# netease-youdao/EmotiVoice

Measured on AMD Instinct MI355X. Metric: mel_frames_per_sec, higher is better.
Workload: dtype f16+mxfp4 (fp32-class activations travelling as plane sets; per product one fp16 MFMA on the hi parts + two block-scaled MFMAs for the cross terms: fp4 x fp4 in every generator stage, the decoder's conv-FFN and QKV / output projections, fp4 weights x E5M2 activations in the fused 32-channel k = 3 pa

## Files before the change

emotivoice_amd/csrc/ev_gemm.hip:

```cpp
#include <hip/hip_fp16.h>
#include <stdlib.h>

#include "ev_kernels.h"
#include "ev_mxq.h"

#pragma clang fp contract(off)

namespace ev {

typedef _Float16 half8 __attribute__((ext_vector_type(8)));
typedef float f32x4 __attribute__((ext_vector_type(4)));
typedef float f32x2 __attribute__((ext_vector_type(2)));
typedef _Float16 half2v __attribute__((ext_vector_type(2)));

static constexpr int MAX_SPAN = 64;

__device__ __forceinline__ float max_raw(float a, float b) {
    float r;
    asm("v_max_f32 %0, %1, %2" : "=v"(r) : "v"(a), "v"(b));
    return r;
}
__device__ __forceinline__ float min_raw(float a, float b) {
    float r;
    asm("v_min_f32 %0, %1, %2" : "=v"(r) : "v"(a), "v"(b));
// ... 1933 lines not shown
                else asm volatile("" :: "v"(o.x), "v"(o.y), "v"(o.z), "v"(o.w));
            }
        }
        vmask = vmask_next;
        EV_PAIR_SYNC()
        cur ^= 1;
    }
#undef EV_PAIR_GLOAD
#undef EV_PAIR_SSTORE
#undef EV_PAIR_ROW
#undef EV_PAIR_VROW
#undef EV_PAIR_VLOAD
#undef EV_PAIR_VMASK
}

static size_t pair_lds_bytes(int k, bool twob = false) {
    if (twob) return 2 * (size_t)k * 32 * 64 + 2 * 320 * 64 + 272 * 64;
    return 2 * (size_t)k * 32 * 64 + 2 * 384 * 64 + 272 * 64 + 8 * 32 * (32 * 4 + 16);
}
static constexpr size_t PAIR64_LDS_BYTES = 2 * 2 * (size_t)(3 * 64 * 64) + 2 * 2 * (size_t)(272 * 64) + 2 * (size_t)(272 * 64);

static int g_n_cu[64];
static bool g_dev_ready[64];
static int current_device() { int d = 0; (void)hipGetDevice(&d); return (d >= 0 && d < 64) ? d : 0; }

static int device_cus() {
    const int d = current_device();
    if (!g_dev_ready[d]) (void)init_device_kernels(d);
    return g_n_cu[d] > 0 ? g_n_cu[d] : 256;
}

void launch_resblock_pair_c32(const ResPairParams& p, hipStream_t s) {
    const int n_cu = device_cus();
    const int h2 = (p.k - 1) / 2, bmo = 256 - 2 * h2;
    const int ntiles = (p.M + bmo - 1) / bmo;
    const int grid = ntiles < n_cu ? ntiles : n_cu;
    static const char* one_env = tuning_env("EV_PAIR_1B");
    const bool twob = p.k <= 3 && !(one_env && one_env[0] == '1') && !(p.epi.reserved0 & 4) && ntiles >= 4 * n_cu;
    const size_t lds = pair_lds_bytes(p.k, twob);
    const int grid2 = ntiles < 2 * n_cu ? ntiles : 2 * n_cu;
#define EV_PAIR_LAUNCH(KK, TB, G)                                                                                          \
        if (p.epi.add16_a) hipLaunchKernelGGL((resblock_pair_c32_kernel<KK, 2, TB>), dim3(G), dim3(512), lds, s, p);  \
        else if (p.epi.acc32) hipLaunchKernelGGL((resblock_pair_c32_kernel<KK, 1, TB>), dim3(G), dim3(512), lds, s, p); \
        else hipLaunchKernelGGL((resblock_pair_c32_kernel<KK, 0, TB>), dim3(G), dim3(512), lds, s, p);
    switch (p.k) {
        case 3: if (twob) { EV_PAIR_LAUNCH(3, true, grid2) } else { EV_PAIR_LAUNCH(3, false, grid) } break;
        case 7: EV_PAIR_LAUNCH(7, false, grid) break;
        case 11: EV_PAIR_LAUNCH(11, false, grid) break;
        default: break;
    }
#undef EV_PAIR_LAUNCH
}

template <int K, int ACCMODE>
__global__ __launch_bounds__(512, 1) void resblock_pair_c64_kernel(const ResPairParams p) {
    constexpr int C = 64, H2 = (K - 1) / 2, BMO = 256 - 2 * H2;
    constexpr int XROWS = 272, PLANE = XROWS * 64, XBYTES = 2 * PLANE;
    constexpr int WPL = K * C * 64, WBYTES = 2 * WPL;
    constexpr int EPITCH = C * 4 + 16, EBYTES = 16 * EPITCH;
    constexpr int XCH = (XROWS * 8 + 511) / 512;
    static_assert(8 * EBYTES <= XBYTES && 256 + 2 * 5 * H2 + 2 * H2 <= XROWS && XCH == 5, "LDS aliasing / slab geometry");
    extern __shared__ __attribute__((aligned(16))) char smem[];
    char* W1s = smem;
    char* W2s = smem + WBYTES;
    char* Xa = smem + 2 * WBYTES;
    char* Xt = Xa + 2 * XBYTES;
    const int tid = threadIdx.x, lane = tid & 63, wave = tid >> 6;
    const int fr = lane & 15, fq = lane >> 4;
    const int h1 = H2 * p.dil;
    const int x_pitch = p.ldx * 2;
    const char* xg = reinterpret_cast<const char*>(p.x);
    const int ntiles = (p.M + BMO - 1) / BMO;
    const ConvGemmParams& e = p.epi;
    const int gmin = p.gmax ? p.gmin : 0, gmax = p.gmax ? p.gmax : p.M;

    for (int c = tid; c < K * C * 8; c += 512) {
        const int row = c >> 3, q = c & 7, tap = row >> 6, co = row & 63, plane = q >> 2, part = q & 3;
        const long off = ((long)(co * K + tap) * C) * 2 + q * 16;
        *reinterpret_cast<uint4*>(W1s + plane * WPL + swz(row, part)) = *reinterpret_cast<const uint4*>(reinterpret_cast<const char*>(p.w1) + off);
        *reinterpret_cast<uint4*>(W2s + plane * WPL + swz(row, part)) = *reinterpret_cast<const uint4*>(reinterpret_cast<const char*>(p.w2) + off);
    }
    f32x2 b1v[4][2];
#pragma unroll
    for (int a = 0; a < 4; ++a)
#pragma unroll
        for (int q = 0; q < 2; ++q) b1v[a][q] = f32x2{p.b1[a * 16 + 4 * fq + 2 * q], p.b1[a * 16 + 4 * fq + 2 * q + 1]};
    const int er = lane >> 3, eg = lane & 7, eco = eg * 8;
    const unsigned frbit = 1u << fr, erbit = 1u << er;
    f32x2 b2v[4];
#pragma unroll
    for (int q = 0; q < 4; ++q) b2v[q] = e.bias ? f32x2{e.bias[eco + 2 * q], e.bias[eco + 2 * q + 1]} : f32x2{0.f, 0.f};
    const f32x2 out_scale2 = f32x2{e.out_scale, e.out_scale};
    const bool has_post = e.post_lrelu != 0;
    const f32x2 post_slope2 = f32x2{e.post_slope, e.post_slope};
    const f32x2 slope01 = f32x2{0.1f, 0.1f};
    __half* const o16 = reinterpret_cast<__half*>(e.out16);
    float* const o32a = e.out32_before_post ? e.out32 : nullptr;
    float* const o32b = e.out32_before_post ? nullptr : e.out32;
    char* const trash = g_store_trash + lane * 64;

    const uint8_t* vptr = e.row_valid ? e.row_valid : g_row_always_valid;
    const int vshift = e.row_valid ? e.valid_shift : 31;
#define EV_P64_VROW(TILE) ((TILE) * BMO - H2 + wave * 32 + lane)
#define EV_P64_VLOAD(TILE, DST) { const int g_ = EV_P64_VROW(TILE); DST = vptr[min(max(g_, gmin), gmax - 1) >> vshift]; }
#define EV_P64_VMASK(TILE, SRC) __builtin_amdgcn_ballot_w64((SRC) != 0 && EV_P64_VROW(TILE) >= gmin && EV_P64_VROW(TILE) < gmax)

    uint4 xr[XCH];
    const int xrow = tid >> 3, xq = tid & 7;
    const char* const xgt = xg + xq * 16;
    const int xdst = (xq >> 2) * PLANE + swz(xrow, xq & 3);
    const bool has5 = wave < 2;
#define EV_P64_GLOAD(TILE)                                                                                 \
    {                                                                                                      \
        const int g0_ = (TILE) * BMO - H2 - h1 + xrow;                                                     \
        _Pragma("unroll") for (int i = 0; i < 4; ++i)                                                      \
            xr[i] = *reinterpret_cast<const uint4*>(xgt + (long)min(g0_ + 64 * i, gmax + 63) * x_pitch);    \
        if (has5) xr[4] = *reinterpret_cast<const uint4*>(xgt + (long)min(g0_ + 256, gmax + 63) * x_pitch); \
    }
#define EV_P64_SSTORE(BUF)                                                                                 \
    {                                                                                                      \
        _Pragma("unroll") for (int i = 0; i < 4; ++i)                                                      \
            *reinterpret_cast<uint4*>(Xa + (BUF) * XBYTES + xdst + i * 4096) = lrelu_h8(xr[i], 0.1f);      \
        if (has5) *reinterpret_cast<uint4*>(Xa + (BUF) * XBYTES + xdst + 4 * 4096) = lrelu_h8(xr[4], 0.1f); \
    }

    int tile = blockIdx.x;
    unsigned long long vmask;
    {
        uint8_t vb;
        EV_P64_GLOAD(tile)
        EV_P64_VLOAD(tile, vb)
        EV_P64_SSTORE(0)
        vmask = EV_P64_VMASK(tile, vb);
    }
    __syncthreads();
    int cur = 0;
    const int wrow0 = wave * 32 + fr;
    for (; tile < ntiles; tile += gridDim.x) {
        const int next = min(tile + (int)gridDim.x, ntiles - 1);
        const int m0 = tile * BMO;
        const int t_end = min(m0 + BMO, p.M);
        uint4 resv[2][2];
        float4 accin[2][2][2];
#pragma unroll
        for (int b = 0; b < 2; ++b)
#pragma unroll
            for (int it = 0; it < 2; ++it) {
                const int t = min(m0 + wave * 32 + b * 16 + it * 8 + er, t_end - 1);
                resv[b][it] = *reinterpret_cast<const uint4*>(xg + (long)t * x_pitch + eg * 16);
                if constexpr (ACCMODE == 1) {
                    const float* ap = e.acc32 + (long)t * e.ldacc + eco;
                    accin[b][it][0] = *reinterpret_cast<const float4*>(ap);
                    accin[b][it][1] = *reinterpret_cast<const float4*>(ap + 4);
                }
                if constexpr (ACCMODE == 2) {
                    *reinterpret_cast<uint4*>(&accin[b][it][0]) = *reinterpret_cast<const uint4*>(reinterpret_cast<const __half*>(e.add16_a) + (long)t * e.ldadd + eco);
                    *reinterpret_cast<uint4*>(&accin[b][it][1]) = *reinterpret_cast<const uint4*>(reinterpret_cast<const __half*>(e.add16_b) + (long)t * e.ldadd + eco);
                }
            }
        uint8_t vb_next;
        EV_P64_GLOAD(next)
        EV_P64_VLOAD(next, vb_next)
        __builtin_amdgcn_sched_barrier(0);
        f32x4 acc[4][2];
#pragma unroll
        for (int a = 0; a < 4; ++a)
#pragma unroll
            for (int b = 0; b < 2; ++b) acc[a][b] = f32x4{0.f, 0.f, 0.f, 0.f};
        {
            const char* Xb = Xa + cur * XBYTES;
#pragma unroll
            for (int t = 0; t < K; ++t) {
                const int r0 = wrow0 + t * p.dil;
                const int xo = r0 * 64 + ((fq ^ ((r0 >> 1) & 3)) << 4);
#pragma unroll
                for (int kc = 0; kc < 2; ++kc) {
                    uint4 xf[2], wf[4];
#pragma unroll
                    for (int b = 0; b < 2; ++b) xf[b] = *reinterpret_cast<const uint4*>(Xb + kc * PLANE + xo + b * 16 * 64);
#pragma unroll
                    for (int a = 0; a < 4; ++a) wf[a] = *reinterpret_cast<const uint4*>(W1s + kc * WPL + swz(t * 64 + a * 16 + fr, fq));
#pragma unroll
                    for (int a = 0; a < 4; ++a)
#pragma unroll
                        for (int b = 0; b < 2; ++b)
                            acc[a][b] = __builtin_amdgcn_mfma_f32_16x16x32_f16(*reinterpret_cast<half8*>(&wf[a]),
                                                                               *reinterpret_cast<half8*>(&xf[b]), acc[a][b], 0, 0, 0);
                }
            }
        }
        const unsigned xtmask = (unsigned)vmask;
#pragma unroll
        for (int b = 0; b < 2; ++b) {
            const int r1 = wrow0 + b * 16;
            const bool valid = (xtmask & (frbit << (b * 16))) != 0u;
#pragma unroll
            for (int a = 0; a < 4; ++a) {
                const f32x2 lo = lrelu2(f32x2{acc[a][b][0], acc[a][b][1]} + b1v[a][0], slope01);
                const f32x2 hi = lrelu2(f32x2{acc[a][b][2], acc[a][b][3]} + b1v[a][1], slope01);
                uint2 w;
                *reinterpret_cast<half2v*>(&w.x) = __builtin_convertvector(lo, half2v);
                *reinterpret_cast<half2v*>(&w.y) = __builtin_convertvector(hi, half2v);
                w.x = valid ? w.x : 0u; w.y = valid ? w.y : 0u;
                const int c32 = (a & 1) * 16 + 4 * fq;
                *reinterpret_cast<uint2*>(Xt + (a >> 1) * PLANE + swz(r1, c32 >> 3) + (c32 & 7) * 2) = w;
            }
        }
        __syncthreads();
#pragma unroll
        for (int a = 0; a < 4; ++a)
#pragma unroll
            for (int b = 0; b < 2; ++b) acc[a][b] = f32x4{0.f, 0.f, 0.f, 0.f};
#pragma unroll
        for (int t = 0; t < K; ++t) {
            const int r0 = wrow0 + t;
            const int xo = r0 * 64 + ((fq ^ ((r0 >> 1) & 3)) << 4);
#pragma unroll
            for (int kc = 0; kc < 2; ++kc) {
                uint4 xf[2], wf[4];
#pragma unroll
                for (int b = 0; b < 2; ++b) xf[b] = *reinterpret_cast<const uint4*>(Xt + kc * PLANE + xo + b * 16 * 64);
#pragma unroll
                for (int a = 0; a < 4; ++a) wf[a] = *reinterpret_cast<const uint4*>(W2s + kc * WPL + swz(t * 64 + a * 16 + fr, fq));
#pragma unroll
                for (int a = 0; a < 4; ++a)
#pragma unroll
                    for (int b = 0; b < 2; ++b)
                        acc[a][b] = __builtin_amdgcn_mfma_f32_16x16x32_f16(*reinterpret_cast<half8*>(&wf[a]),
                                                                           *reinterpret_cast<half8*>(&xf[b]), acc[a][b], 0, 0, 0);
            }
        }
        __builtin_amdgcn_sched_barrier(0);
        EV_P64_SSTORE(cur ^ 1)
        const unsigned long long vmask_next = EV_P64_VMASK(next, vb_next);
        char* es = Xa + cur * XBYTES + wave * EBYTES;
        const unsigned outmask = (unsigned)(vmask >> H2);
#pragma unroll
        for (int b = 0; b < 2; ++b) {
            __builtin_amdgcn_wave_barrier();
#pragma unroll
            for (int a = 0; a < 4; ++a)
                *reinterpret_cast<f32x4*>(es + fr * EPITCH + (a * 16 + 4 * fq) * 4) = acc[a][b];
            __builtin_amdgcn_wave_barrier();
#pragma unroll
            for (int it = 0; it < 2; ++it) {
                const int lr = it * 8 + er;
                const int t = m0 + wave * 32 + b * 16 + lr;
                const bool rowok = t < t_end;
                const bool valid = (outmask & (erbit << (b * 16 + it * 8))) != 0u;
                const f32x4 v0 = *reinterpret_cast<const f32x4*>(es + lr * EPITCH + eg * 32);
                const f32x4 v1 = *reinterpret_cast<const f32x4*>(es + lr * EPITCH + eg * 32 + 16);
                f32x2 v[4] = {f32x2{v0[0], v0[1]}, f32x2{v0[2], v0[3]}, f32x2{v1[0], v1[1]}, f32x2{v1[2], v1[3]}};
                const half2v* hh = reinterpret_cast<const half2v*>(&resv[b][it]);
#pragma unroll
                for (int q = 0; q < 4; ++q) v[q] = (v[q] + b2v[q] + __builtin_convertvector(hh[q], f32x2)) * out_scale2;
                if constexpr (ACCMODE == 1) {
                    v[0] += f32x2{accin[b][it][0].x, accin[b][it][0].y}; v[1] += f32x2{accin[b][it][0].z, accin[b][it][0].w};
                    v[2] += f32x2{accin[b][it][1].x, accin[b][it][1].y}; v[3] += f32x2{accin[b][it][1].z, accin[b][it][1].w};
                }
                if constexpr (ACCMODE == 2) {
                    const half2v* ha = reinterpret_cast<const half2v*>(&accin[b][it][0]);
                    const half2v* hb = reinterpret_cast<const half2v*>(&accin[b][it][1]);
#pragma unroll
                    for (int q = 0; q < 4; ++q) v[q] += __builtin_convertvector(ha[q], f32x2) + __builtin_convertvector(hb[q], f32x2);
                }
                if (o32a) {
                    float* op = rowok ? o32a + (long)t * e.ldo + eco : reinterpret_cast<float*>(trash);
                    *reinterpret_cast<float4*>(op) = valid ? make_float4(v[0][0], v[0][1], v[1][0], v[1][1]) : make_float4(0.f, 0.f, 0.f, 0.f);
                    *reinterpret_cast<float4*>(op + 4) = valid ? make_float4(v[2][0], v[2][1], v[3][0], v[3][1]) : make_float4(0.f, 0.f, 0.f, 0.f);
                }
                if (has_post) {
#pragma unroll
                    for (int q = 0; q < 4; ++q) v[q] = lrelu2(v[q], post_slope2);
                }
                if (o32b) {
                    float* op = rowok ? o32b + (long)t * e.ldo + eco : reinterpret_cast<float*>(trash);
                    *reinterpret_cast<float4*>(op) = valid ? make_float4(v[0][0], v[0][1], v[1][0], v[1][1]) : make_float4(0.f, 0.f, 0.f, 0.f);
                    *reinterpret_cast<float4*>(op + 4) = valid ? make_float4(v[2][0], v[2][1], v[3][0], v[3][1]) : make_float4(0.f, 0.f, 0.f, 0.f);
                }
                if (o16) {
                    uint4 o;
                    half2v* h = reinterpret_cast<half2v*>(&o);
#pragma unroll
                    for (int q = 0; q < 4; ++q) h[q] = __builtin_convertvector(v[q], half2v);
                    o.x = valid ? o.x : 0u; o.y = valid ? o.y : 0u; o.z = valid ? o.z : 0u; o.w = valid ? o.w : 0u;
                    *reinterpret_cast<uint4*>(rowok ? reinterpret_cast<char*>(o16 + (long)t * e.ldo + eco) : trash) = o;
                }
            }
        }
        vmask = vmask_next;
        __syncthreads();
        cur ^= 1;
    }
#undef EV_P64_GLOAD
#undef EV_P64_SSTORE
#undef EV_P64_VROW
#undef EV_P64_VLOAD
#undef EV_P64_VMASK
}

#include "ev_gemm_mx.h"
#include "ev_gemm_mx64.h"
#include "ev_pair_mx.h"
#include "ev_pair_e5.h"

#include "ev_conv64_mx.h"
#include "ev_pair64_mx.h"

int init_device_kernels(int device) {
    if (device < 0 || device >= 64) return -1;
    hipDeviceProp_t prop;
    if (hipGetDeviceProperties(&prop, device) != hipSuccess) return -1;
    g_n_cu[device] = prop.multiProcessorCount > 0 ? prop.multiProcessorCount : 256;
    hipError_t e = hipSuccess;
    auto attr = [&](const void* fn, size_t bytes) { const hipError_t r = hipFuncSetAttribute(fn, hipFuncAttributeMaxDynamicSharedMemorySize, (int)bytes); if (r != hipSuccess) e = r; };
#define EV_PAIR_ATTR(KK, TB)                                                             \
    attr((const void*)resblock_pair_c32_kernel<KK, 0, TB>, pair_lds_bytes(KK, TB));      \
    attr((const void*)resblock_pair_c32_kernel<KK, 1, TB>, pair_lds_bytes(KK, TB));      \
    attr((const void*)resblock_pair_c32_kernel<KK, 2, TB>, pair_lds_bytes(KK, TB));
    EV_PAIR_ATTR(3, false) EV_PAIR_ATTR(7, false) EV_PAIR_ATTR(11, false) EV_PAIR_ATTR(3, true)
#undef EV_PAIR_ATTR
    attr((const void*)resblock_pair_c64_kernel<3, 0>, PAIR64_LDS_BYTES);
    attr((const void*)resblock_pair_c64_kernel<3, 1>, PAIR64_LDS_BYTES);
    attr((const void*)resblock_pair_c64_kernel<3, 2>, PAIR64_LDS_BYTES);
    if (x3_set_attributes() != hipSuccess) e = hipErrorInvalidValue;
    if (phased_set_attributes() != hipSuccess) e = hipErrorInvalidValue;
    if (mx_set_attributes() != hipSuccess) e = hipErrorInvalidValue;
    if (mx64_set_attributes() != hipSuccess) e = hipErrorInvalidValue;
    if (pair_mx_set_attributes() != hipSuccess) e = hipErrorInvalidValue;
    if (pair_e5_set_attributes() != hipSuccess) e = hipErrorInvalidValue;
    if (conv64_mx_set_attributes() != hipSuccess) e = hipErrorInvalidValue;
    if (pair64_mx_set_attributes() != hipSuccess) e = hipErrorInvalidValue;
    g_dev_ready[device] = (e == hipSuccess);
    return e == hipSuccess ? 0 : -1;
}
int launch_resblock_pair_c32_mx(const ResPairParams& p, hipStream_t s) {
    const ConvGemmParams& e = p.epi;
    if (!p.w1_mx || !p.w2_mx || !e.out32 || e.out16 || e.add16_a || e.post_lrelu || e.seq_bias || e.mxo_h || !(p.k == 3 || p.k == 7 || p.k == 11) ||
        (p.k - 1) / 2 * (p.dil + 1) * 2 + 256 > 320 || p.ldx != 32) return -1;
    const int n_cu = device_cus();
    const int h2 = (p.k - 1) / 2;
    if (!(e.reserved0 & 16) && (p.k == 3 || (e.reserved0 & 32))) {
        const int bmo2 = 128 - 2 * h2, ntiles2 = (p.M + bmo2 - 1) / bmo2;
        const int grid2 = (ntiles2 + 1) / 2 < n_cu ? (ntiles2 + 1) / 2 : n_cu;
#define EV_PE5_LAUNCH(KK)                                                                                                           \
        if (e.acc32) hipLaunchKernelGGL((resblock_pair_c32_e5_kernel<KK, 1>), dim3(grid2), dim3(512), PairE5Geom<KK>::TOTAL, s, p);   \
        else hipLaunchKernelGGL((resblock_pair_c32_e5_kernel<KK, 0>), dim3(grid2), dim3(512), PairE5Geom<KK>::TOTAL, s, p);
        switch (p.k) {
            case 3: EV_PE5_LAUNCH(3) break;
            case 7: EV_PE5_LAUNCH(7) break;
            default: EV_PE5_LAUNCH(11) break;
        }
#undef EV_PE5_LAUNCH
        return 0;
    }
    {
        const int bmo2 = 128 - 2 * h2, ntiles2 = (p.M + bmo2 - 1) / bmo2;
        if (!(e.reserved0 & 4) && ntiles2 >= 2) {
            const int grid2 = (ntiles2 + 1) / 2 < n_cu ? (ntiles2 + 1) / 2 : n_cu;
#define EV_PMX2_LAUNCH(KK)                                                                                                          \
            if (e.acc32) hipLaunchKernelGGL((resblock_pair_c32_mx2_kernel<KK, 1>), dim3(grid2), dim3(512), PairMx2Geom<KK>::TOTAL, s, p);   \
            else hipLaunchKernelGGL((resblock_pair_c32_mx2_kernel<KK, 0>), dim3(grid2), dim3(512), PairMx2Geom<KK>::TOTAL, s, p);
            switch (p.k) {
                case 3: EV_PMX2_LAUNCH(3) break;
                case 7: EV_PMX2_LAUNCH(7) break;
                default: EV_PMX2_LAUNCH(11) break;
            }
#undef EV_PMX2_LAUNCH
            return 0;
        }
    }
    const int bmo = 256 - 2 * h2;
    const int ntiles = (p.M + bmo - 1) / bmo;
    const int grid = ntiles < n_cu ? ntiles : n_cu;
#define EV_PMX_LAUNCH(KK)                                                                                                         \
        if (e.acc32) hipLaunchKernelGGL((resblock_pair_c32_mx_kernel<KK, 1>), dim3(grid), dim3(512), PairMxGeom<KK>::TOTAL, s, p);   \
        else hipLaunchKernelGGL((resblock_pair_c32_mx_kernel<KK, 0>), dim3(grid), dim3(512), PairMxGeom<KK>::TOTAL, s, p);
    switch (p.k) {
        case 3: EV_PMX_LAUNCH(3) break;
        case 7: EV_PMX_LAUNCH(7) break;
        default: EV_PMX_LAUNCH(11) break;
    }
#undef EV_PMX_LAUNCH
    return 0;
}

void launch_resblock_pair_c64(const ResPairParams& p, hipStream_t s) {
    const size_t bytes = PAIR64_LDS_BYTES;
    const int n_cu = device_cus();
    const int bmo = 256 - 2;
    const int ntiles = (p.M + bmo - 1) / bmo;
    const int grid = ntiles < n_cu ? ntiles : n_cu;
    if (p.epi.add16_a) hipLaunchKernelGGL((resblock_pair_c64_kernel<3, 2>), dim3(grid), dim3(512), bytes, s, p);
    else if (p.epi.acc32) hipLaunchKernelGGL((resblock_pair_c64_kernel<3, 1>), dim3(grid), dim3(512), bytes, s, p);
    else hipLaunchKernelGGL((resblock_pair_c64_kernel<3, 0>), dim3(grid), dim3(512), bytes, s, p);
}

int mx_launch_kind(const ConvGemmParams& p) {
    if (p.dtype != DT_MX) return 0;
    return (mx64_eligible(p) || conv64_mx_eligible(p)) ? 2 : (mx_eligible(p) ? 1 : 0);
}

int splitk_check(const ConvGemmParams& p) {
    if (p.ksplit <= 1) return 0;
    if (p.dtype != DT_F32S || p.ksplit > 16 || p.N % 64 || p.K % 32 || (p.K / 32) % p.ksplit || p.M % 128 || p.add16_a || (!p.out32 && !p.out16)) return -1;
    if (!p.mx_scratch || ((uintptr_t)p.mx_scratch & 15) || p.mx_scratch_size < (size_t)p.ksplit * (size_t)p.M * (size_t)p.N * 4) return -1;
    return 0;
}

void launch_conv_gemm(const ConvGemmParams& p, hipStream_t s) {
    (void)device_cus();
    if (p.dtype == DT_F16) launch_dt<_Float16>(p, s);
    else if (p.dtype == DT_F32S) launch_split(p, s);
    else if (p.dtype == DT_MX) {
        if (mx64_eligible(p)) launch_mx64(p, s);
        else if (conv64_mx_eligible(p)) launch_conv64_mx(p, s);
        else if (mx_eligible(p)) launch_mx(p, s);
        else { ConvGemmParams q = p; q.dtype = DT_F32S; launch_split(q, s); }
    } else launch_dt<float>(p, s);
}

}
```

Measured before the change: 722,000.

## Add register-resident-weight fused resblock pair kernel for k=11 (and opt-in k=7)

Adds a new fused two-conv resblock kernel for 32-channel k=11 (and k=7 behind a flag). Each wave holds its fp16 hi-part weights in registers, and for k<=7 the fp4 cross-term weights too, instead of rereading them from LDS. The two conv stages are split across wave groups with double-buffered LDS tiles, so the second conv overlaps the first conv of the next tile. It trades higher register pressure and a fixed 256-row tile for fewer LDS weight reads, and replaces the previous mx2 path for k=11 by default.

After: 728,200, median of 6. About the same (+0.9%).

```diff
diff --git a/emotivoice_amd/csrc/ev_gemm.hip b/emotivoice_amd/csrc/ev_gemm.hip
--- a/emotivoice_amd/csrc/ev_gemm.hip
+++ b/emotivoice_amd/csrc/ev_gemm.hip
@@ -2259,6 +2259,7 @@
 #include "ev_gemm_mx.h"
 #include "ev_gemm_mx64.h"
 #include "ev_pair_mx.h"
+#include "ev_pair_regw.h"
 #include "ev_pair_e5.h"
 
 #include "ev_conv64_mx.h"
@@ -2285,6 +2286,7 @@
     if (mx_set_attributes() != hipSuccess) e = hipErrorInvalidValue;
     if (mx64_set_attributes() != hipSuccess) e = hipErrorInvalidValue;
     if (pair_mx_set_attributes() != hipSuccess) e = hipErrorInvalidValue;
+    if (pair_regw_set_attributes() != hipSuccess) e = hipErrorInvalidValue;
     if (pair_e5_set_attributes() != hipSuccess) e = hipErrorInvalidValue;
     if (conv64_mx_set_attributes() != hipSuccess) e = hipErrorInvalidValue;
     if (pair64_mx_set_attributes() != hipSuccess) e = hipErrorInvalidValue;
@@ -2311,6 +2313,16 @@
 #undef EV_PE5_LAUNCH
         return 0;
     }
+    if (!(e.reserved0 & (4 | 8 | 64)) && (p.k == 11 || (p.k == 7 && (e.reserved0 & 128)))) {
+        const int bmo = 256 - 2 * h2, ntiles = (p.M + bmo - 1) / bmo;
+        const int grid = ntiles < n_cu ? ntiles : n_cu;
+#define EV_PRW_LAUNCH(KK)                                                                                                           \
+        if (e.acc32) hipLaunchKernelGGL((resblock_pair_c32_regw_kernel<KK, 1, PairRwCfg<KK>::WQREG>), dim3(grid), dim3(512), (PairRwGeom<KK, PairRwCfg<KK>::WQREG>::TOTAL), s, p);   \
+        else hipLaunchKernelGGL((resblock_pair_c32_regw_kernel<KK, 0, PairRwCfg<KK>::WQREG>), dim3(grid), dim3(512), (PairRwGeom<KK, PairRwCfg<KK>::WQREG>::TOTAL), s, p);
+        if (p.k == 7) { EV_PRW_LAUNCH(7) } else { EV_PRW_LAUNCH(11) }
+#undef EV_PRW_LAUNCH
+        return 0;
+    }
     {
         const int bmo2 = 128 - 2 * h2, ntiles2 = (p.M + bmo2 - 1) / bmo2;
         if (!(e.reserved0 & 4) && ntiles2 >= 2) {
diff --git a/emotivoice_amd/csrc/ev_pair_regw.h b/emotivoice_amd/csrc/ev_pair_regw.h
--- /dev/null
+++ b/emotivoice_amd/csrc/ev_pair_regw.h
@@ -0,0 +1,349 @@
+#pragma once
+
+template <int K, bool WQREG>
+struct PairRwGeom {
+    static constexpr int C = 32, H2 = (K - 1) / 2, BMO = 256 - 2 * H2, KG = (K + 3) / 4, KP = KG * 4;
+    static constexpr int XR = 320, TR = 272, EPITCH = C * 4 + 16;
+    static constexpr int WQB = KP * C * 16, WSB = KP * C;
+    static constexpr int XB = XR * 64 + 2 * XR * 16 + 2 * XR;
+    static constexpr int TB = TR * 64 + 2 * TR * 16 + 2 * TR;
+    static constexpr int OFF_WQ = 0, OFF_WS = WQREG ? 0 : 4 * WQB, OFF_X = WQREG ? 0 : 4 * WQB + 4 * WSB;
+    static constexpr int OFF_T = OFF_X + 2 * XB, OFF_ES = OFF_T + 2 * TB;
+    static constexpr int TOTAL = OFF_ES + 4 * 16 * EPITCH;
+    static_assert(OFF_X % 16 == 0 && XB % 16 == 0 && TB % 16 == 0 && OFF_ES % 16 == 0 && TOTAL <= 160 * 1024 && 256 + K - 1 <= TR, "LDS plan");
+};
+
+template <int K, int ACCMODE, bool WQREG>
+__global__ __launch_bounds__(512, 1) void resblock_pair_c32_regw_kernel(const ResPairParams p) {
+    using G = PairRwGeom<K, WQREG>;
+    constexpr int C = G::C, H2 = G::H2, BMO = G::BMO, KG = G::KG, XR = G::XR, TR = G::TR, EPITCH = G::EPITCH;
+    extern __shared__ __attribute__((aligned(16))) char smem[];
+    const int tid = threadIdx.x, lane = tid & 63;
+    const int wave = __builtin_amdgcn_readfirstlane(tid >> 6);
+    const int gi = wave >> 2, lw = wave & 3, ltid = tid & 255;
+    const int fr = lane & 15, fq = lane >> 4;
+    const int dil = p.dil, h1 = H2 * dil;
+    const int x_pitch = p.ldx * 4;
+    const char* xg = reinterpret_cast<const char*>(p.x);
+    const int ntiles = (p.M + BMO - 1) / BMO;
+    const ConvGemmParams& e = p.epi;
+    const int gmin = p.gmax ? p.gmin : 0, gmax = p.gmax ? p.gmax : p.M;
+#define EV_PRW_XH(buf) (smem + G::OFF_X + (buf) * G::XB)
+#define EV_PRW_TH(buf) (smem + G::OFF_T + (buf) * G::TB)
+
+    const char* const whg = reinterpret_cast<const char*>(gi ? p.w2 : p.w1);
+    const char* const wmg = reinterpret_cast<const char*>(gi ? p.w2_mx : p.w1_mx);
+    uint4 wh[K][2];
+#pragma unroll
+    for (int t = 0; t < K; ++t)
+#pragma unroll
+        for (int a = 0; a < 2; ++a) wh[t][a] = *reinterpret_cast<const uint4*>(whg + ((long)((a * 16 + fr) * K + t) * C) * 2 + fq * 16);
+    uint4 wq[WQREG ? KG : 1][2][2];
+    int ws[WQREG ? KG : 1][2][2];
+    if constexpr (WQREG) {
+#pragma unroll
+        for (int g = 0; g < KG; ++g)
+#pragma unroll
+            for (int pl = 0; pl < 2; ++pl)
+#pragma unroll
+                for (int a = 0; a < 2; ++a) {
+                    const int wrow = (4 * g + fq) * 32 + a * 16 + fr;
+                    wq[g][pl][a] = *reinterpret_cast<const uint4*>(wmg + pl * G::WQB + wrow * 16);
+                    ws[g][pl][a] = *reinterpret_cast<const uint8_t*>(wmg + 2 * G::WQB + pl * G::WSB + wrow);
+                }
+    } else {
+        char* const Wq = smem + G::OFF_WQ;
+        char* const Wsc = smem + G::OFF_WS;
+        for (int c = tid; c < 2 * G::WQB / 16; c += 512) {
+            *reinterpret_cast<uint4*>(Wq + c * 16) = *reinterpret_cast<const uint4*>(reinterpret_cast<const char*>(p.w1_mx) + c * 16);
+            *reinterpret_cast<uint4*>(Wq + 2 * G::WQB + c * 16) = *reinterpret_cast<const uint4*>(reinterpret_cast<const char*>(p.w2_mx) + c * 16);
+        }
+        for (int c = tid; c < 2 * G::WSB / 16; c += 512) {
+            *reinterpret_cast<uint4*>(Wsc + c * 16) = *reinterpret_cast<const uint4*>(reinterpret_cast<const char*>(p.w1_mx) + 2 * G::WQB + c * 16);
+            *reinterpret_cast<uint4*>(Wsc + 2 * G::WSB + c * 16) = *reinterpret_cast<const uint4*>(reinterpret_cast<const char*>(p.w2_mx) + 2 * G::WQB + c * 16);
+        }
+    }
+    const f32x2 slope01 = f32x2{0.1f, 0.1f};
+    const uint8_t* vptr = e.row_valid ? e.row_valid : g_row_always_valid;
+    const int vshift = e.row_valid ? e.valid_shift : 31;
+#define EV_PRW_VLOAD(G0, DST) { const int g_ = (G0) + lane; DST = vptr[min(max(g_, gmin), gmax - 1) >> vshift]; }
+#define EV_PRW_VMASK(G0, SRC) __builtin_amdgcn_ballot_w64((SRC) != 0 && (G0) + lane >= gmin && (G0) + lane < gmax)
+
+#define EV_PRW_CONV(XH, NR, DIL, MID)                                                                         \
+    {                                                                                                      \
+        const int wrow0 = (int)vlane((unsigned)wrow0_inv);           \
+        const char* const xq_base_ = (XH) + (NR) * 64;                                                     \
+        const char* const xs_base_ = xq_base_ + 2 * (NR) * 16;                                             \
+        uint4 xf_[2][4];           \
+        _Pragma("unroll") for (int b = 0; b < 4; ++b)                                                      \
+            xf_[0][b] = *reinterpret_cast<const uint4*>((XH) + wrow0 * 64 + ((fq ^ ((wrow0 >> 1) & 3)) << 4) + b * 16 * 64); \
+        _Pragma("unroll") for (int t = 0; t < K; ++t) {                                                    \
+            if (t + 1 < K) {                                                                               \
+                const int r0 = wrow0 + (t + 1) * (DIL);                                                    \
+                const char* xp = (XH) + r0 * 64 + ((fq ^ ((r0 >> 1) & 3)) << 4);                           \
+                _Pragma("unroll") for (int b = 0; b < 4; ++b) xf_[(t + 1) & 1][b] = *reinterpret_cast<const uint4*>(xp + b * 16 * 64); \
+            }                                                                                              \
+            _Pragma("unroll") for (int b = 0; b < 4; ++b)                                                  \
+                _Pragma("unroll") for (int a = 0; a < 2; ++a)                                              \
+                    acc[a][b] = __builtin_amdgcn_mfma_f32_16x16x32_f16(*reinterpret_cast<half8*>(&wh[t][a]), *reinterpret_cast<half8*>(&xf_[t & 1][b]), acc[a][b], 0, 0, 0); \
+            __builtin_amdgcn_sched_barrier(0);                                                             \
+        }                                                                                                  \
+        MID                                                                                                \
+        __builtin_amdgcn_sched_barrier(0);                                                                 \
+        _Pragma("unroll") for (int g = 0; g < KG; ++g) {                                                   \
+            const int tw = 4 * g + fq;                      \
+            const int rq = wrow0 + min(tw, K - 1) * (DIL);  \
+            _Pragma("unroll") for (int pl = 0; pl < 2; ++pl) {                                             \
+                uint4 wq_[2], xq_[4];                                                                      \
+                int ws_[2], xs_[4];                                                                        \
+                _Pragma("unroll") for (int a = 0; a < 2; ++a) {                                            \
+                    if constexpr (WQREG) { wq_[a] = wq[g][pl][a]; ws_[a] = ws[g][pl][a]; }                 \
+                    else {                                                                                 \
+                        wq_[a] = *reinterpret_cast<const uint4*>(smem + G::OFF_WQ + (gi * 2 + pl) * G::WQB + (tw * 32 + a * 16 + fr) * 16); \
+                        ws_[a] = *reinterpret_cast<const uint8_t*>(smem + G::OFF_WS + (gi * 2 + pl) * G::WSB + tw * 32 + a * 16 + fr); \
+                    }                                                                                      \
+                }                                                                                          \
+                _Pragma("unroll") for (int b = 0; b < 4; ++b) {                                            \
+                    xq_[b] = *reinterpret_cast<const uint4*>(xq_base_ + pl * (NR) * 16 + (rq + b * 16) * 16); \
+                    xs_[b] = *reinterpret_cast<const uint8_t*>(xs_base_ + pl * (NR) + rq + b * 16);        \
+                }                                                                                          \
+                _Pragma("unroll") for (int b = 0; b < 4; ++b)                                              \
+                    _Pragma("unroll") for (int a = 0; a < 2; ++a)                                          \
+                        mfma_mx_inplace(acc[a][b], wq_[a], xq_[b], ws_[a], xs_[b]);                        \
+                __builtin_amdgcn_sched_barrier(0);                                                         \
+            }                                                                                              \
+        }                                                                                                  \
+        mfma_asm_fence(acc);                 \
+    }
+#define EV_PRW_BARRIER()                                         \
+    {                                                            \
+        asm volatile("s_waitcnt lgkmcnt(0)" ::: "memory");       \
+        __builtin_amdgcn_sched_barrier(0);                       \
+        __builtin_amdgcn_s_barrier();                            \
+        __builtin_amdgcn_sched_barrier(0);                       \
+    }
+
+    const int niter = (ntiles - (int)blockIdx.x + (int)gridDim.x - 1) / (int)gridDim.x;
+    const int wrow0_inv = lw * 64 + fr;
+
+    if (gi == 0) {
+        f32x2 b1v[2][2];
+#pragma unroll
+        for (int a = 0; a < 2; ++a)
+#pragma unroll
+            for (int q = 0; q < 2; ++q) b1v[a][q] = f32x2{p.b1[a * 16 + 4 * fq + 2 * q], p.b1[a * 16 + 4 * fq + 2 * q + 1]};
+        float4 xr[5][2];
+        const int xq = ltid & 3, xrow = ltid >> 2;
+        const char* const xgt = xg + xq * 32;
+        const bool need5 = lw * 16 < (K - 1) * dil;
+#define EV_PRW_ROW(G_) min((G_), gmax + 63)
+#define EV_PRW_GLOAD(TILE)                                                                                 \
+        _Pragma("unroll") for (int i = 0; i < 5; ++i) if (i < 4 || need5) {                                \
+            const char* q_ = xgt + (long)EV_PRW_ROW((TILE) * BMO - H2 - h1 + xrow + 64 * i) * x_pitch;     \
+            xr[i][0] = *reinterpret_cast<const float4*>(q_); xr[i][1] = *reinterpret_cast<const float4*>(q_ + 16); \
+        }
+#define EV_PRW_SSTORE(BUF)                                                                                 \
+        {                                                                                                  \
+            char* const Xh_ = EV_PRW_XH(BUF);                                                              \
+            char* const Xq_ = Xh_ + XR * 64;                                                               \
+            char* const Xs_ = Xq_ + 2 * XR * 16;                                                           \
+            const int xrow_ = (int)vlane((unsigned)xrow);           \
+            _Pragma("unroll") for (int i = 0; i < 5; ++i) if (i < 4 || need5) {                            \
+                const int drow_ = xrow_ + 64 * i;                                                          \
+                f32x2 a_[4] = {lrelu2(f32x2{xr[i][0].x, xr[i][0].y}, slope01), lrelu2(f32x2{xr[i][0].z, xr[i][0].w}, slope01), \
+                               lrelu2(f32x2{xr[i][1].x, xr[i][1].y}, slope01), lrelu2(f32x2{xr[i][1].z, xr[i][1].w}, slope01)}; \
+                uint4 ho_; unsigned ch_, cl_, bh_, bl_;                                                    \
+                mx_quant8(a_, ho_, ch_, cl_, bh_, bl_);                                                    \
+                *reinterpret_cast<uint4*>(Xh_ + swz(drow_, xq)) = ho_;                                     \
+                *reinterpret_cast<unsigned*>(Xq_ + drow_ * 16 + xq * 4) = ch_;                             \
+                *reinterpret_cast<unsigned*>(Xq_ + XR * 16 + drow_ * 16 + xq * 4) = cl_;                   \
+                if (xq == 0) { Xs_[drow_] = (char)bh_; Xs_[XR + drow_] = (char)bl_; }                      \
+                __builtin_amdgcn_sched_barrier(0);           \
+            }                                                                                              \
+        }
+        const unsigned long long frbit = 1ull << fr;
+        int tile = blockIdx.x;
+        unsigned long long vmask;
+        {
+            uint8_t vb;
+            EV_PRW_GLOAD(tile)
+            EV_PRW_VLOAD(tile * BMO - H2 + lw * 64, vb)
+            EV_PRW_SSTORE(0)
+            vmask = EV_PRW_VMASK(tile * BMO - H2 + lw * 64, vb);
+        }
+        EV_PRW_BARRIER()
+        for (int it_ = 0; it_ < niter; ++it_, tile += (int)gridDim.x) {
+            const int buf = it_ & 1;
+            const int next = min(tile + (int)gridDim.x, ntiles - 1);
+            uint8_t vb_next;
+#define EV_PRW_A_MID int next_ = next; asm volatile("" : "+s"(next_)); EV_PRW_GLOAD(next_) EV_PRW_VLOAD(next_ * BMO - H2 + lw * 64, vb_next)
+            f32x4 acc[2][4];
+#pragma unroll
+            for (int a = 0; a < 2; ++a)
+#pragma unroll
+                for (int b = 0; b < 4; ++b) acc[a][b] = f32x4{0.f, 0.f, 0.f, 0.f};
+            EV_PRW_CONV(EV_PRW_XH(buf), XR, dil, EV_PRW_A_MID)
+#undef EV_PRW_A_MID
+            char* const Th = EV_PRW_TH(buf);
+            char* const Tq = Th + TR * 64;
+            char* const Tsc = Tq + 2 * TR * 16;
+            const int wrow0 = (int)vlane((unsigned)wrow0_inv);
+            const bool xt_masked = vmask != ~0ull;
+#pragma unroll
+            for (int b = 0; b < 4; ++b) {
+                const int r1 = wrow0 + b * 16;
+                const bool valid = (vmask & (frbit << (b * 16))) != 0ull;
+                f32x2 v[2][2];
+                half2v hh[2][2];
+                f32x2 hf[2][2], lf[2][2];
+                float mh = 0.f, ml = 0.f;
+#pragma unroll
+                for (int a = 0; a < 2; ++a) {
+                    v[a][0] = lrelu2(f32x2{acc[a][b][0], acc[a][b][1]} + b1v[a][0], slope01);
+                    v[a][1] = lrelu2(f32x2{acc[a][b][2], acc[a][b][3]} + b1v[a][1], slope01);
+#pragma unroll
+                    for (int q = 0; q < 2; ++q) {
+                        if (xt_masked) { v[a][q][0] = valid ? v[a][q][0] : 0.f; v[a][q][1] = valid ? v[a][q][1] : 0.f; }
+                        hh[a][q] = __builtin_convertvector(v[a][q], half2v);
+                        hf[a][q] = __builtin_convertvector(hh[a][q], f32x2);
+                        lf[a][q] = v[a][q] - hf[a][q];
+                        mh = max3_abs_raw(hf[a][q][0], hf[a][q][1], mh);
+                        ml = max3_abs_raw(lf[a][q][0], lf[a][q][1], ml);
+                    }
+                }
+                mh = max_xor16_raw(max_xor32_raw(mh));
+                ml = max_xor16_raw(max_xor32_raw(ml));
+                const unsigned bh = mx_scale_byte(mh), bl = mx_scale_byte(ml);
+                const float sh = __uint_as_float(bh << 23), sl = __uint_as_float(bl << 23);
+#pragma unroll
+                for (int a = 0; a < 2; ++a) {
+                    uint2 w;
+                    w.x = *reinterpret_cast<unsigned*>(&hh[a][0]); w.y = *reinterpret_cast<unsigned*>(&hh[a][1]);
+                    const int co = a * 16 + 4 * fq;
+                    *reinterpret_cast<uint2*>(Th + swz(r1, co >> 3) + (co & 7) * 2) = w;
+                    unsigned ch = 0, cl = 0;
+                    ch = __builtin_amdgcn_cvt_scalef32_pk_fp4_f32(ch, hf[a][0][0], hf[a][0][1], sh, 0);
+                    ch = __builtin_amdgcn_cvt_scalef32_pk_fp4_f32(ch, hf[a][1][0], hf[a][1][1], sh, 1);
+                    cl = __builtin_amdgcn_cvt_scalef32_pk_fp4_f32(cl, lf[a][0][0], lf[a][0][1], sl, 0);
+                    cl = __builtin_amdgcn_cvt_scalef32_pk_fp4_f32(cl, lf[a][1][0], lf[a][1][1], sl, 1);
+                    *reinterpret_cast<unsigned short*>(Tq + r1 * 16 + (co >> 1)) = (unsigned short)ch;
+                    *reinterpret_cast<unsigned short*>(Tq + TR * 16 + r1 * 16 + (co >> 1)) = (unsigned short)cl;
+                }
+                if (fq == 0) { Tsc[r1] = (char)bh; Tsc[TR + r1] = (char)bl; }
+                __builtin_amdgcn_sched_barrier(0);
+            }
+            EV_PRW_SSTORE(buf ^ 1)
+            vmask = EV_PRW_VMASK(next * BMO - H2 + lw * 64, vb_next);
+            EV_PRW_BARRIER()
+        }
+#undef EV_PRW_SSTORE
+#undef EV_PRW_GLOAD
+#undef EV_PRW_ROW
+    } else {
+        char* const es = smem + G::OFF_ES + lw * 16 * EPITCH;
+        const int er = lane >> 2, eg = lane & 3, eco = eg * 8;
+        f32x2 b2v[4];
+#pragma unroll
+        for (int q = 0; q < 4; ++q) b2v[q] = e.bias ? f32x2{e.bias[eco + 2 * q], e.bias[eco + 2 * q + 1]} : f32x2{0.f, 0.f};
+        const f32x2 out_scale2 = f32x2{e.out_scale, e.out_scale};
+        float* const o32 = e.out32;
+        char* const trash = g_store_trash + lane * 64;
+        const unsigned long long erbit = 1ull << er;
+        EV_PRW_BARRIER()
+        EV_PRW_BARRIER()
+        int tile = blockIdx.x;
+        for (int it_ = 0; it_ < niter; ++it_, tile += (int)gridDim.x) {
+            const int buf = it_ & 1;
+            const int m0 = tile * BMO;
+            const int t_end = min(m0 + BMO, p.M);
+            float4 resv[4][2], accin[4][2];
+            uint8_t vb;
+#define EV_PRW_B_MID                                                                                       \
+            int m0m = m0;                                                                                  \
+            asm volatile("" : "+s"(m0m));           \
+            _Pragma("unroll") for (int it = 0; it < 4; ++it) {                                             \
+                const int t = min(m0m + lw * 64 + it * 16 + er, min(m0m + BMO, p.M) - 1);                  \
+                const char* rp = xg + (long)t * x_pitch + eg * 32;                                         \
+                resv[it][0] = *reinterpret_cast<const float4*>(rp);                                        \
+                resv[it][1] = *reinterpret_cast<const float4*>(rp + 16);                                   \
+                if (ACCMODE == 1 && it < 2) {           \
+                    const float* ap = e.acc32 + (long)t * e.ldacc + eco;                                   \
+                    accin[it][0] = *reinterpret_cast<const float4*>(ap);                                   \
+                    accin[it][1] = *reinterpret_cast<const float4*>(ap + 4);                               \
+                }                                                                                          \
+            }                                                                                              \
+            EV_PRW_VLOAD(m0m + lw * 64, vb)
+            f32x4 acc[2][4];
+#pragma unroll
+            for (int a = 0; a < 2; ++a)
+#pragma unroll
+                for (int b = 0; b < 4; ++b) acc[a][b] = f32x4{0.f, 0.f, 0.f, 0.f};
+            EV_PRW_CONV(EV_PRW_TH(buf), TR, 1, EV_PRW_B_MID)
+#undef EV_PRW_B_MID
+            const unsigned long long outmask = EV_PRW_VMASK(m0 + lw * 64, vb);
+            int m0e = m0;
+            asm volatile("" : "+s"(m0e));
+            if constexpr (ACCMODE == 1) {
+#pragma unroll
+                for (int it = 2; it < 4; ++it) {
+                    const float* ap = e.acc32 + (long)min(m0e + lw * 64 + it * 16 + er, t_end - 1) * e.ldacc + eco;
+                    accin[it][0] = *reinterpret_cast<const float4*>(ap);
+                    accin[it][1] = *reinterpret_cast<const float4*>(ap + 4);
+                }
+            }
+#pragma unroll
+            for (int it = 0; it < 4; ++it) {
+                const int t = m0e + lw * 64 + it * 16 + er;
+                const bool rowok = t < t_end;
+                const bool valid = (outmask & (erbit << (it * 16))) != 0ull;
+                __builtin_amdgcn_wave_barrier();
+#pragma unroll
+                for (int a = 0; a < 2; ++a) *reinterpret_cast<f32x4*>(es + fr * EPITCH + (a * 16 + 4 * fq) * 4) = acc[a][it];
+                __builtin_amdgcn_wave_barrier();
+                const f32x4 v0 = *reinterpret_cast<const f32x4*>(es + er * EPITCH + eg * 32);
+                const f32x4 v1 = *reinterpret_cast<const f32x4*>(es + er * EPITCH + eg * 32 + 16);
+                f32x2 v[4] = {f32x2{v0[0], v0[1]}, f32x2{v0[2], v0[3]}, f32x2{v1[0], v1[1]}, f32x2{v1[2], v1[3]}};
+                const f32x2 rr[4] = {f32x2{resv[it][0].x, resv[it][0].y}, f32x2{resv[it][0].z, resv[it][0].w},
+                                     f32x2{resv[it][1].x, resv[it][1].y}, f32x2{resv[it][1].z, resv[it][1].w}};
+#pragma unroll
+                for (int q = 0; q < 4; ++q) v[q] = (v[q] + b2v[q] + rr[q]) * out_scale2;
+                if constexpr (ACCMODE == 1) {
+                    v[0] += f32x2{accin[it][0].x, accin[it][0].y}; v[1] += f32x2{accin[it][0].z, accin[it][0].w};
+                    v[2] += f32x2{accin[it][1].x, accin[it][1].y}; v[3] += f32x2{accin[it][1].z, accin[it][1].w};
+                }
+                float* op = rowok ? o32 + (long)t * e.ldo + eco : reinterpret_cast<float*>(trash);
+                if (outmask == ~0ull) {
+                    *reinterpret_cast<float4*>(op) = make_float4(v[0][0], v[0][1], v[1][0], v[1][1]);
+                    *reinterpret_cast<float4*>(op + 4) = make_float4(v[2][0], v[2][1], v[3][0], v[3][1]);
+                } else {
+                    *reinterpret_cast<float4*>(op) = valid ? make_float4(v[0][0], v[0][1], v[1][0], v[1][1]) : make_float4(0.f, 0.f, 0.f, 0.f);
+                    *reinterpret_cast<float4*>(op + 4) = valid ? make_float4(v[2][0], v[2][1], v[3][0], v[3][1]) : make_float4(0.f, 0.f, 0.f, 0.f);
+                }
+            }
+            if (it_ + 1 < niter) EV_PRW_BARRIER()
+        }
+    }
+#undef EV_PRW_BARRIER
+#undef EV_PRW_CONV
+#undef EV_PRW_VLOAD
+#undef EV_PRW_VMASK
+#undef EV_PRW_XH
+#undef EV_PRW_TH
+}
+
+template <int K> struct PairRwCfg { static constexpr bool WQREG = K <= 7; };
+
+template <int K>
+static hipError_t pair_regw_attr() {
+    constexpr bool WQ = PairRwCfg<K>::WQREG;
+    hipError_t e = hipSuccess, r;
+    r = hipFuncSetAttribute((const void*)resblock_pair_c32_regw_kernel<K, 0, WQ>, hipFuncAttributeMaxDynamicSharedMemorySize, PairRwGeom<K, WQ>::TOTAL); if (r != hipSuccess) e = r;
+    r = hipFuncSetAttribute((const void*)resblock_pair_c32_regw_kernel<K, 1, WQ>, hipFuncAttributeMaxDynamicSharedMemorySize, PairRwGeom<K, WQ>::TOTAL); if (r != hipSuccess) e = r;
+    return e;
+}
+static hipError_t pair_regw_set_attributes() {
+    hipError_t e = hipSuccess, r;
+    r = pair_regw_attr<7>(); if (r != hipSuccess) e = r;
+    r = pair_regw_attr<11>(); if (r != hipSuccess) e = r;
+    return e;
+}
```
